# guy3540/Acoustic_Locating_VQ-VAE

Hardware: AMD Instinct MI355X
Metric: spectrograms/sec (train step), speech VQ-VAE default config (higher is better)
Workload: dtype x3mx_hb

## Files before the change

### acoustic_locating_vq-vae_amd/csrc/conv1d_bf16_k3.hip

```cpp
#include <stdlib.h>

#include "alvq_common.h"
#include "bf16_common.h"
#include "conv1d_bf16_tile256.h"

namespace alvq {

constexpr int K3_XSLAB = 17 * 1024;
constexpr int K3_STAGE = 3 * V2_HALF + K3_XSLAB;
constexpr int K3_LDS = 2 * K3_STAGE;
static_assert(V2_EPI_LDS <= K3_LDS, "C slab must fit");

template <int OUT, int F16 = 0>
__global__ __launch_bounds__(512, 2) void conv1d_bf16_k3_kernel(ConvBArgs a) {
  extern __shared__ __attribute__((aligned(16))) unsigned char lds[];
  const int tid = threadIdx.x, lane = tid & 63;
  const int wave = __builtin_amdgcn_readfirstlane(tid >> 6);
  const int li = lane & 15, kq = lane >> 4;
  const int wm0 = (wave >> 2) * 128, wn0 = (wave & 3) * 64;

  const int tile = xcd_remap(blockIdx.x, a.mtiles * a.rtiles);
  const int m0 = (tile % a.mtiles) * V2_M;
  const int r0 = (tile / a.mtiles) * V2_R;
  const int Cp = a.Cp;

  const int hsel = (lane >> 4) & 3;
  const int hval = (hsel == 0) ? 0 : (4 - hsel);
  const int srow = lane >> 2, sgrp = (lane & 3) ^ hval;
  const unsigned lane_off = (unsigned)(srow * Cp + sgrp * 8) * 2u;
  const unsigned lane_off_x = (unsigned)(srow * Cp + ((lane & 3) ^ ((hsel & 1) * 2)) * 8) * 2u;
  const long tap_w = (long)a.Mp128 * Cp;
  const long row16 = (long)Cp * 32;
  const unsigned lds0 = (unsigned)(unsigned long)((__attribute__((address_space(3))) unsigned char*)lds);
  auto dma = [&](const char* sbase, unsigned lds_dst) {
    asm volatile("s_mov_b32 m0, %2\n\ts_nop 0\n\tglobal_load_lds_dwordx4 %0, %1" ::"v"(lane_off), "s"(sbase), "s"(lds_dst)
                 : "memory");
  };
  auto dma_x = [&](const char* sbase, unsigned lds_dst) {
    asm volatile("s_mov_b32 m0, %2\n\ts_nop 0\n\tglobal_load_lds_dwordx4 %0, %1" ::"v"(lane_off_x), "s"(sbase), "s"(lds_dst)
                 : "memory");
  };
  const char* const wA = (const char*)(a.wp + (wave >> 2) * tap_w + ((long)m0 + (wave & 3) * 64) * Cp);
  const unsigned dA = lds0 + (wave >> 2) * V2_HALF + (wave & 3) * 4096;
  const char* const wB = (const char*)(a.wp + 2 * tap_w + ((long)m0 + wave * 32) * Cp);
  const char* const xB = (const char*)(a.x + ((long)r0 - 1 + wave * 32) * Cp);
  const unsigned dBw = lds0 + 2 * V2_HALF + wave * 2048, dBx = lds0 + 3 * V2_HALF + wave * 2048;

  auto issueA = [&](int c) {
    const unsigned dst = (c & 1) * K3_STAGE + dA;
    const char* ws = wA + c * (V2_K * 2);
    dma(ws, dst);
    dma(ws + row16, dst + 1024);
    dma(ws + 2 * row16, dst + 2048);
    dma(ws + 3 * row16, dst + 3072);
  };
  auto issueB = [&](int c) {
    const unsigned st = (c & 1) * K3_STAGE;
    const char* ws = wB + c * (V2_K * 2);
    const char* xs = xB + c * (V2_K * 2);
    dma(ws, st + dBw);
    dma(ws + row16, st + dBw + 1024);
    dma_x(xs, st + dBx);
    dma_x(xs + row16, st + dBx + 1024);
    if (wave == 7 && srow < 2) dma_x(xs + 2 * row16, st + dBx + 2048);
  };

  const int hl = (li >> 2) & 3;
  const int loffA = li * 64 + ((kq ^ (hl == 0 ? 0 : 4 - hl)) << 4);
  int loffX[3];
#pragma unroll
  for (int t = 0; t < 3; ++t) {
    const int r = li + t;
    loffX[t] = r * 64 + ((kq ^ (((r >> 2) & 1) * 2)) << 4);
  }
  const unsigned char* const abase = lds + wm0 * 64 + loffA;
  const unsigned char* const xbase = lds + 3 * V2_HALF + wn0 * 64;
  bf16x8_t fa[8], fb[2][4];
  auto rdA = [&](int half, int stage, int tap) {
    const unsigned char* pa = abase + stage * K3_STAGE + tap * V2_HALF;
#pragma unroll
    for (int mi = half * 4; mi < half * 4 + 4; ++mi) fa[mi] = *(const bf16x8_t*)(pa + mi * 1024);
  };
  auto rdB = [&](int q, int stage, int tap) {
    const unsigned char* pb = xbase + stage * K3_STAGE + loffX[tap];
#pragma unroll
    for (int ni = 0; ni < 4; ++ni) fb[q][ni] = *(const bf16x8_t*)(pb + ni * 1024);
  };

  f32x4 acc[8][4];
#pragma unroll
  for (int i = 0; i < 8; ++i)
#pragma unroll
    for (int j = 0; j < 4; ++j) acc[i][j] = f32x4{0.f, 0.f, 0.f, 0.f};
  auto mm = [&](int q, int half) {
#pragma unroll
    for (int mi = half * 4; mi < half * 4 + 4; ++mi)
#pragma unroll
      for (int ni = 0; ni < 4; ++ni)
        if (F16) asm("v_mfma_f32_16x16x32_f16 %0, %1, %2, %0" : "+v"(acc[mi][ni]) : "v"(fa[mi]), "v"(fb[q][ni]));
        else asm("v_mfma_f32_16x16x32_bf16 %0, %1, %2, %0" : "+v"(acc[mi][ni]) : "v"(fa[mi]), "v"(fb[q][ni]));
  };

  const int nch = Cp / V2_K;
  const bool early = wave < 4;

  issueA(0);
  issueB(0);
  issueA(1);
  asm volatile("s_waitcnt vmcnt(4)" ::: "memory");
  __builtin_amdgcn_s_barrier();
  rdA(0, 0, 0);
  rdA(1, 0, 0);
  rdB(0, 0, 0);

#define ALVQ_K3_PHASE(Q, NS, NT, DMA)                    \
  if (early) { DMA; }                                    \
  mm(Q, 0);                                              \
  __builtin_amdgcn_sched_barrier(0);                     \
  rdA(0, NS, NT);                                        \
  rdB((Q) ^ 1, NS, NT);                                  \
  __builtin_amdgcn_sched_barrier(0);                     \
  if (!early) { DMA; }                                   \
  mm(Q, 1);                                              \
  __builtin_amdgcn_sched_barrier(0);                     \
  rdA(1, NS, NT);                                        \
  __builtin_amdgcn_sched_barrier(0);

#define ALVQ_K3_CHUNK(c, S, Q0)                                                   \
  ALVQ_K3_PHASE(Q0, S, 1, if ((c) + 1 < nch) issueB((c) + 1))                     \
  ALVQ_K3_PHASE((Q0) ^ 1, S, 2, (void)0)                                          \
  asm volatile("s_waitcnt vmcnt(0) lgkmcnt(0)" ::: "memory");                     \
  __builtin_amdgcn_s_barrier();                                                   \
  ALVQ_K3_PHASE(Q0, (S) ^ 1, 0, if ((c) + 2 < nch) issueA((c) + 2))

  for (int c = 0; c < nch; c += 2) {
    ALVQ_K3_CHUNK(c, 0, 0)
    ALVQ_K3_CHUNK(c + 1, 1, 1)
  }
#undef ALVQ_K3_CHUNK
#undef ALVQ_K3_PHASE
  asm volatile("s_nop 15\n\ts_nop 15" ::: "memory");
  __syncthreads();

  tile256_epilogue<OUT, F16>(a, acc, lds, m0, r0, wave, tid, li, kq, wm0);
}

int conv1d_bf16_k3_launch(const ConvBArgs& a_in, hipStream_t stream) {
  ConvBArgs a = a_in;
  const long rows = (long)a.rtiles * TB_R;
  a.rtiles = (int)(rows / V2_R);
  a.mtiles = (a.M + V2_M - 1) / V2_M;
  static DeviceOnce attr;
  if (attr.need()) {
    (void)hipFuncSetAttribute((const void*)conv1d_bf16_k3_kernel<0>, hipFuncAttributeMaxDynamicSharedMemorySize, K3_LDS);
    (void)hipFuncSetAttribute((const void*)conv1d_bf16_k3_kernel<1>, hipFuncAttributeMaxDynamicSharedMemorySize, K3_LDS);
    (void)hipFuncSetAttribute((const void*)conv1d_bf16_k3_kernel<0, 1>, hipFuncAttributeMaxDynamicSharedMemorySize, K3_LDS);
    (void)hipFuncSetAttribute((const void*)conv1d_bf16_k3_kernel<1, 1>, hipFuncAttributeMaxDynamicSharedMemorySize, K3_LDS);
  }
  const dim3 grid(a.rtiles * a.mtiles), block(512);
  if (a.elem) {
    if (a.y) hipLaunchKernelGGL((conv1d_bf16_k3_kernel<0, 1>), grid, block, K3_LDS, stream, a);
    else hipLaunchKernelGGL((conv1d_bf16_k3_kernel<1, 1>), grid, block, K3_LDS, stream, a);
  } else if (a.y) hipLaunchKernelGGL((conv1d_bf16_k3_kernel<0>), grid, block, K3_LDS, stream, a);
  else hipLaunchKernelGGL((conv1d_bf16_k3_kernel<1>), grid, block, K3_LDS, stream, a);
  return check_launch("alvq_conv1d_bf16(k3)");
}

}
```

### acoustic_locating_vq-vae_amd/csrc/conv1d_bf16_tile256.h

```cpp
#pragma once
#include "bf16_common.h"

namespace alvq {

constexpr int V2_M = 256, V2_R = 256, V2_K = 32;
constexpr int V2_HALF = V2_M * V2_K * 2;
constexpr int V2_CS = V2_M + 4;
constexpr int V2_EPI_LDS = 64 * V2_CS * 4;

struct FragSet {
  bf16x8_t a[8];
  bf16x8_t b[4];
};

template <int NMI, int NNI, int F16 = 0>
__device__ __forceinline__ void wave_epilogue_bf16(const ConvBArgs& a, const f32x4 (&acc)[NMI][NNI], int m0, int r0, int li,
                                                   int kq, int wm0, int wn0);

template <int OUT, int F16 = 0>
__device__ __forceinline__ void tile256_epilogue(const ConvBArgs& a, const f32x4 (&acc)[8][4], unsigned char* lds, int m0,
                                                 int r0, int wave, int tid, int li, int kq, int wm0) {
  if (OUT == 0) {
    wave_epilogue_bf16<8, 4, F16>(a, acc, m0, r0, li, kq, wm0, (wave & 3) * 64);
    return;
  }
  const float oscale = a.out_scale ? *a.out_scale : 1.f;
  float* Cs = (float*)lds;
  const int Lp1 = a.L + 1, ndata = a.B * Lp1;
  for (int slab = 0; slab < 4; ++slab) {
    if ((wave & 3) == slab) {
#pragma unroll
      for (int mi = 0; mi < 8; ++mi)
#pragma unroll
        for (int ni = 0; ni < 4; ++ni) {
          const int rl = ni * 16 + li, ml = wm0 + mi * 16 + kq * 4;
          *(f32x4*)(Cs + rl * V2_CS + ml) = acc[mi][ni];
        }
    }
    __syncthreads();
    const int rl = tid & 63, row = r0 + slab * 64 + rl;
    int b, l;
    if (row_valid(row, Lp1, ndata, &b, &l)) {
      for (int ml = tid >> 6; ml < V2_M; ml += 8) {
        const int m = m0 + ml;
        if (m >= a.M) break;
        a.y_ncl[((long)b * a.M + m) * a.L + l] = (Cs[rl * V2_CS + ml] + (a.bias ? a.bias[m] : 0.f)) * oscale;
      }
    }
    __syncthreads();
  }
}

template <int NMI, int NNI, int F16>
__device__ __forceinline__ void wave_epilogue_bf16(const ConvBArgs& a, const f32x4 (&acc)[NMI][NNI], int m0, int r0, int li,
                                                   int kq, int wm0, int wn0) {
  static_assert(NMI % 2 == 0, "fragments are swapped in pairs");
  elem_saturate<F16>();
  unsigned watch = 0;
  const int Lp1 = a.L + 1, ndata = a.B * Lp1;
  const int mb0 = m0 + wm0 + (kq & 1) * 16 + (kq >> 1) * 8;
#pragma unroll
  for (int ni = 0; ni < NNI; ++ni) {
    const int row = r0 + wn0 + ni * 16 + li;
    int b, l;
    const bool ok = row_valid(row, Lp1, ndata, &b, &l);
    const bool gaps = !__all(ok);
    const long o0 = (long)row * a.Mop + mb0;
    u16x8 s1[NMI / 2], s2[NMI / 2], mk[NMI / 2];
#pragma unroll
    for (int mp = 0; mp < NMI; mp += 2) {
      if (m0 + wm0 + mp * 16 >= a.Mop) continue;
      if (a.skip1) s1[mp / 2] = *(const u16x8*)(a.skip1 + o0 + mp * 16);
      if (a.skip2) s2[mp / 2] = *(const u16x8*)(a.skip2 + o0 + mp * 16);
      if (a.mask && !a.mask_bits) mk[mp / 2] = *(const u16x8*)(a.mask + o0 + mp * 16);
    }
    __builtin_amdgcn_sched_barrier(0);
#pragma unroll
    for (int mp = 0; mp < NMI; mp += 2) {
      if (m0 + wm0 + mp * 16 >= a.Mop) continue;
      const long o = o0 + mp * 16;
      const int mb = mb0 + mp * 16;
      float v[8];
#pragma unroll
      for (int e = 0; e < 4; ++e) {
        const u32x2 r = __builtin_amdgcn_permlane16_swap(__float_as_uint(acc[mp][ni][e]), __float_as_uint(acc[mp + 1][ni][e]),
                                                         false, false);
        v[e] = __uint_as_float(r[0]);
        v[e + 4] = __uint_as_float(r[1]);
      }
      if (a.bias) {
        if (m0 + wm0 + mp * 16 + 32 <= a.M) {
          const f32x4 b0 = *(const f32x4*)(a.bias + mb), b1 = *(const f32x4*)(a.bias + mb + 4);
#pragma unroll
          for (int e = 0; e < 4; ++e) {
            v[e] += b0[e];
            v[4 + e] += b1[e];
          }
        } else {
#pragma unroll
          for (int e = 0; e < 8; ++e) v[e] += (mb + e < a.M) ? a.bias[mb + e] : 0.f;
        }
      }
      if (a.skip1) {
#pragma unroll
        for (int e = 0; e < 8; ++e) v[e] += elem2f<F16>(s1[mp / 2][e]);
      }
      if (a.skip2) {
#pragma unroll
        for (int e = 0; e < 8; ++e) v[e] += elem2f<F16>(s2[mp / 2][e]);
      }
      if (a.relu & 1) {
#pragma unroll
        for (int e = 0; e < 8; ++e) v[e] = fmaxf(v[e], 0.f);
      }
      if (a.mask_bits) {
        const int bt = (int)a.mask_bits[o >> 3];
#pragma unroll
        for (int e = 0; e < 8; ++e) v[e] = __uint_as_float(__float_as_uint(v[e]) & (unsigned)((bt << (31 - e)) >> 31));
      } else if (a.mask) {
#pragma unroll
        for (int e = 0; e < 8; ++e) v[e] = (short)mk[mp / 2][e] > 0 ? v[e] : 0.f;
      }
      u32x4 out;
#pragma unroll
      for (int e = 0; e < 4; ++e) out[e] = elem_pk<F16>(v[2 * e], v[2 * e + 1]);
      if (gaps) {
#pragma unroll
        for (int e = 0; e < 4; ++e) out[e] = ok ? out[e] : 0u;
      }
      *(u32x4*)(a.y + o) = out;
      if (F16) {
#pragma unroll
        for (int e = 0; e < 4; ++e) fp16_watch(watch, out[e]);
      }
      if (a.y2) {
        const u16x8 ps = *(const u16x8*)(a.post + o);
        u32x4 out2;
#pragma unroll
        for (int e = 0; e < 4; ++e) out2[e] = elem_pk<F16>(v[2 * e] + elem2f<F16>(ps[2 * e]), v[2 * e + 1] + elem2f<F16>(ps[2 * e + 1]));
        if (gaps) {
#pragma unroll
          for (int e = 0; e < 4; ++e) out2[e] = ok ? out2[e] : 0u;
        }
        *(u32x4*)(a.y2 + o) = out2;
      }
      if (a.bits_out) {
        unsigned bt = 0;
#pragma unroll
        for (int e = 7; e >= 0; --e) {
          const int half = (int)((e & 1) ? (out[e >> 1] & 0xffff0000u) : (out[e >> 1] << 16));
          const int t = half > 0 ? half : 0;
          bt = __builtin_amdgcn_alignbit(bt, 0u - (unsigned)t, 31);
        }
        a.bits_out[o >> 3] = (unsigned char)bt;
      }
    }
  }
  if (F16) fp16_report(watch, a.range_flag);
}

}
```

### acoustic_locating_vq-vae_amd/csrc/conv1d_bf16_v2.hip

```cpp
#include "alvq_common.h"
#include "bf16_common.h"
#include "conv1d_bf16_tile256.h"

namespace alvq {

constexpr int V2_STAGE = 2 * V2_HALF;
constexpr int V2_NSTAGE = 4;
constexpr int V2_LDS = V2_NSTAGE * V2_STAGE;
static_assert(V2_EPI_LDS <= V2_LDS, "C slab must fit");

template <int OUT, int F16 = 0>
__global__ __launch_bounds__(512, 2) void conv1d_bf16_v2_kernel(ConvBArgs a, int KW) {
  extern __shared__ __attribute__((aligned(16))) unsigned char lds[];
  const int PAD = (KW - 1) / 2;
  const int tid = threadIdx.x, lane = tid & 63;
  const int wave = __builtin_amdgcn_readfirstlane(tid >> 6);
  const int li = lane & 15, kq = lane >> 4;
  const int wm0 = (wave >> 2) * 128, wn0 = (wave & 3) * 64;

  const int tile = xcd_remap(blockIdx.x, a.mtiles * a.rtiles);
  const int m0 = (tile % a.mtiles) * V2_M;
  const int r0 = (tile / a.mtiles) * V2_R;
  const int Cp = a.Cp;

  const int hsel = (lane >> 4) & 3;
  const int hval = (hsel == 0) ? 0 : (4 - hsel);
  const int srow = lane >> 2, sgrp = (lane & 3) ^ hval;
  const long lane_off = (long)srow * Cp + sgrp * 8;
  const u16* const wbase = a.wp + ((long)m0 + wave * 32) * Cp + lane_off;
  const u16* const xbase = a.x + ((long)r0 - PAD + wave * 32) * Cp + lane_off;
  const long tap_w = (long)a.Mp128 * Cp;

  int is_chunk = 0, is_tap = 0;
  auto issue = [&](int stage) {
    unsigned char* dst = lds + stage * V2_STAGE + wave * 2048;
    const u16* ws = wbase + is_tap * tap_w + is_chunk * V2_K;
    const u16* xs = xbase + (long)is_tap * Cp + is_chunk * V2_K;
    glds16(ws, dst);
    glds16(ws + 16L * Cp, dst + 1024);
    glds16(xs, dst + V2_HALF);
    glds16(xs + 16L * Cp, dst + V2_HALF + 1024);
    if (++is_tap == KW) {
      is_tap = 0;
      ++is_chunk;
    }
  };

  const int loff = li * 64 + ((kq ^ ((((li >> 2) & 3) == 0) ? 0 : (4 - ((li >> 2) & 3)))) << 4);
  const unsigned char* const abase = lds + wm0 * 64 + loff;
  const unsigned char* const bbase = lds + V2_HALF + wn0 * 64 + loff;
  auto rd = [&](FragSet& f, int stage) {
    const unsigned char* pa = abase + stage * V2_STAGE;
    const unsigned char* pb = bbase + stage * V2_STAGE;
#pragma unroll
    for (int mi = 0; mi < 8; ++mi) f.a[mi] = *(const bf16x8_t*)(pa + mi * 1024);
#pragma unroll
    for (int ni = 0; ni < 4; ++ni) f.b[ni] = *(const bf16x8_t*)(pb + ni * 1024);
  };

  f32x4 acc[8][4];
#pragma unroll
  for (int i = 0; i < 8; ++i)
#pragma unroll
    for (int j = 0; j < 4; ++j) acc[i][j] = f32x4{0.f, 0.f, 0.f, 0.f};
  auto mm = [&](const FragSet& f, int half) {
#pragma unroll
    for (int mi = half * 4; mi < half * 4 + 4; ++mi)
#pragma unroll
      for (int ni = 0; ni < 4; ++ni)
        acc[mi][ni] = elem_mfma16<F16>(f.a[mi], f.b[ni], acc[mi][ni]);
  };

  const int n = (Cp / V2_K) * KW;
  const bool early = wave < 4;
  FragSet f0, f1;

  issue(0);
  issue(1);
  if (n > 2) {
    issue(2);
    asm volatile("s_waitcnt vmcnt(8)" ::: "memory");
  } else {
    asm volatile("s_waitcnt vmcnt(4)" ::: "memory");
  }
  __builtin_amdgcn_s_barrier();
  rd(f0, 0);
  if (n > 2) {
    asm volatile("s_waitcnt vmcnt(4)" ::: "memory");
  } else {
    asm volatile("s_waitcnt vmcnt(0)" ::: "memory");
  }
  __builtin_amdgcn_s_barrier();

  for (int t = 0; t < n; t += 2) {
    if (t + 3 < n && early) issue((t + 3) & 3);
    mm(f0, 0);
    __builtin_amdgcn_sched_barrier(0);
    rd(f1, (t + 1) & 3);
    __builtin_amdgcn_sched_barrier(0);
    if (t + 3 < n && !early) issue((t + 3) & 3);
    mm(f0, 1);
    if (t + 3 < n) {
      asm volatile("s_waitcnt vmcnt(4)" ::: "memory");
    } else {
      asm volatile("s_waitcnt vmcnt(0)" ::: "memory");
    }
    __builtin_amdgcn_s_barrier();
    if (t + 4 < n && early) issue((t + 4) & 3);
    mm(f1, 0);
    __builtin_amdgcn_sched_barrier(0);
    if (t + 2 < n) rd(f0, (t + 2) & 3);
    __builtin_amdgcn_sched_barrier(0);
    if (t + 4 < n && !early) issue((t + 4) & 3);
    mm(f1, 1);
    if (t + 4 < n) {
      asm volatile("s_waitcnt vmcnt(4)" ::: "memory");
    } else {
      asm volatile("s_waitcnt vmcnt(0)" ::: "memory");
    }
    __builtin_amdgcn_s_barrier();
  }

  tile256_epilogue<OUT, F16>(a, acc, lds, m0, r0, wave, tid, li, kq, wm0);
}

int conv1d_bf16_v2_launch(const ConvBArgs& a_in, int KW, hipStream_t stream) {
  ConvBArgs a = a_in;
  const long rows = (long)a.rtiles * TB_R;
  a.rtiles = (int)(rows / V2_R);
  a.mtiles = (a.M + V2_M - 1) / V2_M;
  static DeviceOnce attr;
  if (attr.need()) {
    (void)hipFuncSetAttribute((const void*)conv1d_bf16_v2_kernel<0>, hipFuncAttributeMaxDynamicSharedMemorySize, V2_LDS);
    (void)hipFuncSetAttribute((const void*)conv1d_bf16_v2_kernel<1>, hipFuncAttributeMaxDynamicSharedMemorySize, V2_LDS);
    (void)hipFuncSetAttribute((const void*)conv1d_bf16_v2_kernel<0, 1>, hipFuncAttributeMaxDynamicSharedMemorySize, V2_LDS);
    (void)hipFuncSetAttribute((const void*)conv1d_bf16_v2_kernel<1, 1>, hipFuncAttributeMaxDynamicSharedMemorySize, V2_LDS);
  }
  const dim3 grid(a.rtiles * a.mtiles), block(512);
  if (a.elem) {
    if (a.y) hipLaunchKernelGGL((conv1d_bf16_v2_kernel<0, 1>), grid, block, V2_LDS, stream, a, KW);
    else hipLaunchKernelGGL((conv1d_bf16_v2_kernel<1, 1>), grid, block, V2_LDS, stream, a, KW);
  } else if (a.y) hipLaunchKernelGGL((conv1d_bf16_v2_kernel<0>), grid, block, V2_LDS, stream, a, KW);
  else hipLaunchKernelGGL((conv1d_bf16_v2_kernel<1>), grid, block, V2_LDS, stream, a, KW);
  return check_launch("alvq_conv1d_bf16(v2)");
}

}
```

Baseline: 7695.

## Stagger barrier placement between wave groups and prioritize trailing waves in bf16 conv kernels

Reworks the main loop of the k3 and v2 bf16 conv kernels so the two wave groups (waves 0-3 and 4-7) hit the waitcnt/barrier at different points of the MFMA sequence. The lagging group is also given higher scheduling priority via s_setprio. Both groups now issue their DMA at the same slot instead of splitting it early/late. The intent is to hide barrier stalls behind the other group's MFMAs and keep the matrix units busy. It also drops the final __syncthreads when OUT==0 and adds env-driven debug variants behind a compile flag. The risks are LDS stage hazards from the changed sync positions and a race in the epilogue if the skipped sync mattered.

```diff
diff --git a/acoustic_locating_vq-vae_amd/csrc/conv1d_bf16_k3.hip b/acoustic_locating_vq-vae_amd/csrc/conv1d_bf16_k3.hip
--- a/acoustic_locating_vq-vae_amd/csrc/conv1d_bf16_k3.hip
+++ b/acoustic_locating_vq-vae_amd/csrc/conv1d_bf16_k3.hip
@@ -11,13 +11,14 @@
 constexpr int K3_LDS = 2 * K3_STAGE;
 static_assert(V2_EPI_LDS <= K3_LDS, "C slab must fit");
 
-template <int OUT, int F16 = 0>
-__global__ __launch_bounds__(512, 2) void conv1d_bf16_k3_kernel(ConvBArgs a) {
+template <int OUT, int F16 = 0, int DBG = 0>
+__global__ __launch_bounds__(512, 2) void conv1d_bf16_k3_kernel(ConvBArgs a, int dbg_arg) {
   extern __shared__ __attribute__((aligned(16))) unsigned char lds[];
   const int tid = threadIdx.x, lane = tid & 63;
   const int wave = __builtin_amdgcn_readfirstlane(tid >> 6);
   const int li = lane & 15, kq = lane >> 4;
   const int wm0 = (wave >> 2) * 128, wn0 = (wave & 3) * 64;
+  const int dbg = DBG ? dbg_arg : 0;
 
   const int tile = xcd_remap(blockIdx.x, a.mtiles * a.rtiles);
   const int m0 = (tile % a.mtiles) * V2_M;
@@ -102,7 +103,8 @@
   };
 
   const int nch = Cp / V2_K;
-  const bool early = wave < 4;
+  const bool ahead = wave < 4;
+  if (!ahead) __builtin_amdgcn_s_setprio(1);
 
   issueA(0);
   issueB(0);
@@ -113,25 +115,32 @@
   rdA(1, 0, 0);
   rdB(0, 0, 0);
 
-#define ALVQ_K3_PHASE(Q, NS, NT, DMA)                    \
-  if (early) { DMA; }                                    \
+#define ALVQ_K3_SYNC                                          \
+  if (!(dbg & 4)) {                                           \
+    asm volatile("s_waitcnt vmcnt(0) lgkmcnt(0)" ::: "memory"); \
+    __builtin_amdgcn_s_barrier();                             \
+  }
+#define ALVQ_K3_PHASE(Q, NS, NT, SYNC, DMA)              \
   mm(Q, 0);                                              \
   __builtin_amdgcn_sched_barrier(0);                     \
-  rdA(0, NS, NT);                                        \
-  rdB((Q) ^ 1, NS, NT);                                  \
+  SYNC;                                                  \
+  if (!(dbg & 2)) {                                      \
+    rdA(0, NS, NT);                                      \
+    rdB((Q) ^ 1, NS, NT);                                \
+  }                                                      \
   __builtin_amdgcn_sched_barrier(0);                     \
-  if (!early) { DMA; }                                   \
+  if (!(dbg & 1)) { DMA; }                               \
   mm(Q, 1);                                              \
   __builtin_amdgcn_sched_barrier(0);                     \
-  rdA(1, NS, NT);                                        \
+  if (!(dbg & 2)) rdA(1, NS, NT);                        \
   __builtin_amdgcn_sched_barrier(0);
 
-#define ALVQ_K3_CHUNK(c, S, Q0)                                                   \
-  ALVQ_K3_PHASE(Q0, S, 1, if ((c) + 1 < nch) issueB((c) + 1))                     \
-  ALVQ_K3_PHASE((Q0) ^ 1, S, 2, (void)0)                                          \
-  asm volatile("s_waitcnt vmcnt(0) lgkmcnt(0)" ::: "memory");                     \
-  __builtin_amdgcn_s_barrier();                                                   \
-  ALVQ_K3_PHASE(Q0, (S) ^ 1, 0, if ((c) + 2 < nch) issueA((c) + 2))
+#define ALVQ_K3_CHUNK(c, S, Q0)                                                                   \
+  ALVQ_K3_PHASE(Q0, S, 1, (void)0, if ((c) + 1 < nch) issueB((c) + 1))                            \
+  ALVQ_K3_PHASE((Q0) ^ 1, S, 2, (void)0, (void)0)                                                 \
+  if (!ahead && (c) + 1 < nch) { ALVQ_K3_SYNC }                                                   \
+  ALVQ_K3_PHASE(Q0, (S) ^ 1, 0, if (ahead && (c) + 1 < nch) { ALVQ_K3_SYNC },                     \
+                if ((c) + 2 < nch) issueA((c) + 2))
 
   for (int c = 0; c < nch; c += 2) {
     ALVQ_K3_CHUNK(c, 0, 0)
@@ -139,8 +148,10 @@
   }
 #undef ALVQ_K3_CHUNK
 #undef ALVQ_K3_PHASE
+#undef ALVQ_K3_SYNC
   asm volatile("s_nop 15\n\ts_nop 15" ::: "memory");
-  __syncthreads();
+  if (OUT == 1) __syncthreads();
+  if (dbg & 8) return;
 
   tile256_epilogue<OUT, F16>(a, acc, lds, m0, r0, wave, tid, li, kq, wm0);
 }
@@ -156,13 +167,25 @@
     (void)hipFuncSetAttribute((const void*)conv1d_bf16_k3_kernel<1>, hipFuncAttributeMaxDynamicSharedMemorySize, K3_LDS);
     (void)hipFuncSetAttribute((const void*)conv1d_bf16_k3_kernel<0, 1>, hipFuncAttributeMaxDynamicSharedMemorySize, K3_LDS);
     (void)hipFuncSetAttribute((const void*)conv1d_bf16_k3_kernel<1, 1>, hipFuncAttributeMaxDynamicSharedMemorySize, K3_LDS);
+#ifdef ALVQ_DEBUG_KERNELS
+    (void)hipFuncSetAttribute((const void*)conv1d_bf16_k3_kernel<0, 0, 1>, hipFuncAttributeMaxDynamicSharedMemorySize, K3_LDS);
+    (void)hipFuncSetAttribute((const void*)conv1d_bf16_k3_kernel<0, 1, 1>, hipFuncAttributeMaxDynamicSharedMemorySize, K3_LDS);
+#endif
   }
   const dim3 grid(a.rtiles * a.mtiles), block(512);
+#ifdef ALVQ_DEBUG_KERNELS
+  const int dbg = dg_dbg_env();
+  if (dbg && a.y) {
+    if (a.elem) hipLaunchKernelGGL((conv1d_bf16_k3_kernel<0, 1, 1>), grid, block, K3_LDS, stream, a, dbg);
+    else hipLaunchKernelGGL((conv1d_bf16_k3_kernel<0, 0, 1>), grid, block, K3_LDS, stream, a, dbg);
+    return check_launch("alvq_conv1d_bf16(k3, dbg)");
+  }
+#endif
   if (a.elem) {
-    if (a.y) hipLaunchKernelGGL((conv1d_bf16_k3_kernel<0, 1>), grid, block, K3_LDS, stream, a);
-    else hipLaunchKernelGGL((conv1d_bf16_k3_kernel<1, 1>), grid, block, K3_LDS, stream, a);
-  } else if (a.y) hipLaunchKernelGGL((conv1d_bf16_k3_kernel<0>), grid, block, K3_LDS, stream, a);
-  else hipLaunchKernelGGL((conv1d_bf16_k3_kernel<1>), grid, block, K3_LDS, stream, a);
+    if (a.y) hipLaunchKernelGGL((conv1d_bf16_k3_kernel<0, 1>), grid, block, K3_LDS, stream, a, 0);
+    else hipLaunchKernelGGL((conv1d_bf16_k3_kernel<1, 1>), grid, block, K3_LDS, stream, a, 0);
+  } else if (a.y) hipLaunchKernelGGL((conv1d_bf16_k3_kernel<0>), grid, block, K3_LDS, stream, a, 0);
+  else hipLaunchKernelGGL((conv1d_bf16_k3_kernel<1>), grid, block, K3_LDS, stream, a, 0);
   return check_launch("alvq_conv1d_bf16(k3)");
 }
 
diff --git a/acoustic_locating_vq-vae_amd/csrc/conv1d_bf16_tile256.h b/acoustic_locating_vq-vae_amd/csrc/conv1d_bf16_tile256.h
--- a/acoustic_locating_vq-vae_amd/csrc/conv1d_bf16_tile256.h
+++ b/acoustic_locating_vq-vae_amd/csrc/conv1d_bf16_tile256.h
@@ -1,7 +1,16 @@
 #pragma once
+#include <stdlib.h>
+
 #include "bf16_common.h"
 
 namespace alvq {
+
+#ifdef ALVQ_DEBUG_KERNELS
+inline int dg_dbg_env() {
+  static const int v = getenv("ALVQ_DG_DBG") ? atoi(getenv("ALVQ_DG_DBG")) : 0;
+  return v;
+}
+#endif
 
 constexpr int V2_M = 256, V2_R = 256, V2_K = 32;
 constexpr int V2_HALF = V2_M * V2_K * 2;
diff --git a/acoustic_locating_vq-vae_amd/csrc/conv1d_bf16_v2.hip b/acoustic_locating_vq-vae_amd/csrc/conv1d_bf16_v2.hip
--- a/acoustic_locating_vq-vae_amd/csrc/conv1d_bf16_v2.hip
+++ b/acoustic_locating_vq-vae_amd/csrc/conv1d_bf16_v2.hip
@@ -9,14 +9,15 @@
 constexpr int V2_LDS = V2_NSTAGE * V2_STAGE;
 static_assert(V2_EPI_LDS <= V2_LDS, "C slab must fit");
 
-template <int OUT, int F16 = 0>
-__global__ __launch_bounds__(512, 2) void conv1d_bf16_v2_kernel(ConvBArgs a, int KW) {
+template <int OUT, int F16 = 0, int DBG = 0>
+__global__ __launch_bounds__(512, 2) void conv1d_bf16_v2_kernel(ConvBArgs a, int KW, int dbg_arg) {
   extern __shared__ __attribute__((aligned(16))) unsigned char lds[];
   const int PAD = (KW - 1) / 2;
   const int tid = threadIdx.x, lane = tid & 63;
   const int wave = __builtin_amdgcn_readfirstlane(tid >> 6);
   const int li = lane & 15, kq = lane >> 4;
   const int wm0 = (wave >> 2) * 128, wn0 = (wave & 3) * 64;
+  const int dbg = DBG ? dbg_arg : 0;
 
   const int tile = xcd_remap(blockIdx.x, a.mtiles * a.rtiles);
   const int m0 = (tile % a.mtiles) * V2_M;
@@ -72,8 +73,18 @@
   };
 
   const int n = (Cp / V2_K) * KW;
-  const bool early = wave < 4;
+  const bool ahead = wave < 4;
+  if (!ahead) __builtin_amdgcn_s_setprio(1);
   FragSet f0, f1;
+  auto sync = [&](bool more) {
+    if (dbg & 4) return;
+    if (more) {
+      asm volatile("s_waitcnt vmcnt(4)" ::: "memory");
+    } else {
+      asm volatile("s_waitcnt vmcnt(0)" ::: "memory");
+    }
+    __builtin_amdgcn_s_barrier();
+  };
 
   issue(0);
   issue(1);
@@ -93,33 +104,25 @@
   __builtin_amdgcn_s_barrier();
 
   for (int t = 0; t < n; t += 2) {
-    if (t + 3 < n && early) issue((t + 3) & 3);
     mm(f0, 0);
     __builtin_amdgcn_sched_barrier(0);
-    rd(f1, (t + 1) & 3);
+    if (ahead && t > 0) sync(t + 2 < n);
+    if (!(dbg & 2)) rd(f1, (t + 1) & 3);
     __builtin_amdgcn_sched_barrier(0);
-    if (t + 3 < n && !early) issue((t + 3) & 3);
+    if (t + 3 < n && !(dbg & 1)) issue((t + 3) & 3);
     mm(f0, 1);
-    if (t + 3 < n) {
-      asm volatile("s_waitcnt vmcnt(4)" ::: "memory");
-    } else {
-      asm volatile("s_waitcnt vmcnt(0)" ::: "memory");
-    }
-    __builtin_amdgcn_s_barrier();
-    if (t + 4 < n && early) issue((t + 4) & 3);
+    if (!ahead && t + 1 < n) sync(t + 3 < n);
     mm(f1, 0);
     __builtin_amdgcn_sched_barrier(0);
-    if (t + 2 < n) rd(f0, (t + 2) & 3);
+    if (ahead) sync(t + 3 < n);
+    if (t + 2 < n && !(dbg & 2)) rd(f0, (t + 2) & 3);
     __builtin_amdgcn_sched_barrier(0);
-    if (t + 4 < n && !early) issue((t + 4) & 3);
+    if (t + 4 < n && !(dbg & 1)) issue((t + 4) & 3);
     mm(f1, 1);
-    if (t + 4 < n) {
-      asm volatile("s_waitcnt vmcnt(4)" ::: "memory");
-    } else {
-      asm volatile("s_waitcnt vmcnt(0)" ::: "memory");
-    }
-    __builtin_amdgcn_s_barrier();
+    if (!ahead && t + 2 < n) sync(t + 4 < n);
   }
+  if (OUT == 1) __syncthreads();
+  if (dbg & 8) return;
 
   tile256_epilogue<OUT, F16>(a, acc, lds, m0, r0, wave, tid, li, kq, wm0);
 }
@@ -135,13 +138,25 @@
     (void)hipFuncSetAttribute((const void*)conv1d_bf16_v2_kernel<1>, hipFuncAttributeMaxDynamicSharedMemorySize, V2_LDS);
     (void)hipFuncSetAttribute((const void*)conv1d_bf16_v2_kernel<0, 1>, hipFuncAttributeMaxDynamicSharedMemorySize, V2_LDS);
     (void)hipFuncSetAttribute((const void*)conv1d_bf16_v2_kernel<1, 1>, hipFuncAttributeMaxDynamicSharedMemorySize, V2_LDS);
+#ifdef ALVQ_DEBUG_KERNELS
+    (void)hipFuncSetAttribute((const void*)conv1d_bf16_v2_kernel<0, 0, 1>, hipFuncAttributeMaxDynamicSharedMemorySize, V2_LDS);
+    (void)hipFuncSetAttribute((const void*)conv1d_bf16_v2_kernel<0, 1, 1>, hipFuncAttributeMaxDynamicSharedMemorySize, V2_LDS);
+#endif
   }
   const dim3 grid(a.rtiles * a.mtiles), block(512);
+#ifdef ALVQ_DEBUG_KERNELS
+  const int dbg = dg_dbg_env();
+  if (dbg && a.y) {
+    if (a.elem) hipLaunchKernelGGL((conv1d_bf16_v2_kernel<0, 1, 1>), grid, block, V2_LDS, stream, a, KW, dbg);
+    else hipLaunchKernelGGL((conv1d_bf16_v2_kernel<0, 0, 1>), grid, block, V2_LDS, stream, a, KW, dbg);
+    return check_launch("alvq_conv1d_bf16(v2, dbg)");
+  }
+#endif
   if (a.elem) {
-    if (a.y) hipLaunchKernelGGL((conv1d_bf16_v2_kernel<0, 1>), grid, block, V2_LDS, stream, a, KW);
-    else hipLaunchKernelGGL((conv1d_bf16_v2_kernel<1, 1>), grid, block, V2_LDS, stream, a, KW);
-  } else if (a.y) hipLaunchKernelGGL((conv1d_bf16_v2_kernel<0>), grid, block, V2_LDS, stream, a, KW);
-  else hipLaunchKernelGGL((conv1d_bf16_v2_kernel<1>), grid, block, V2_LDS, stream, a, KW);
+    if (a.y) hipLaunchKernelGGL((conv1d_bf16_v2_kernel<0, 1>), grid, block, V2_LDS, stream, a, KW, 0);
+    else hipLaunchKernelGGL((conv1d_bf16_v2_kernel<1, 1>), grid, block, V2_LDS, stream, a, KW, 0);
+  } else if (a.y) hipLaunchKernelGGL((conv1d_bf16_v2_kernel<0>), grid, block, V2_LDS, stream, a, KW, 0);
+  else hipLaunchKernelGGL((conv1d_bf16_v2_kernel<1>), grid, block, V2_LDS, stream, a, KW, 0);
   return check_launch("alvq_conv1d_bf16(v2)");
 }
 
```

Result: no change. 7689 (median of 6 runs) (-0.1%).
